# pitlover/Monocular-Depth-Estimation

Measured on AMD Instinct MI355X. Metric: images/sec (train step) NYU 640x480 bs=8/GPU, higher is better.
Workload: dtype fp32; 1 GPU; NewCRFs Swin-L (large07) train step, NYU 480x640; model=NewCRFs-L07, global_batch=8, per_gpu_batch=8, num_accum=1, parallelism=dp1, reference_config=json/nyu/newcrfs/newcrfs_github_eval.json, matmul_precision=fp32, hipgraph=False

## Files before the change

### monocular-depth-estimation_amd/csrc/winattn.hip

```cpp
#include "common.h"

namespace mdemi {

struct WinGeom {
  int B, H, W, Hp, Wp, nWh, nWw, shift, heads;
};

template <int WS>
struct Win {
  int b, wy, wx;
  __device__ Win(const WinGeom& g, int win) {
    wx = win % g.nWw;
    const int t = win / g.nWw;
    wy = t % g.nWh;
    b = t / g.nWh;
  }
  __device__ int row(const WinGeom& g, int t) const {
    const int py = wy * WS + t / WS, px = wx * WS + t % WS;
    int oy = py + g.shift, ox = px + g.shift;
    if (oy >= g.Hp) oy -= g.Hp;
    if (ox >= g.Wp) ox -= g.Wp;
    if (oy >= g.H || ox >= g.W) return -1;
    return (b * g.H + oy) * g.W + ox;
  }
  __device__ int region(const WinGeom& g, int t) const {
    const int py = wy * WS + t / WS, px = wx * WS + t % WS;
    const int rh = py < g.Hp - WS ? 0 : (py < g.Hp - g.shift ? 1 : 2);
    const int rw = px < g.Wp - WS ? 0 : (px < g.Wp - g.shift ? 1 : 2);
    return rh * 3 + rw;
  }
};

template <int WS>
__device__ __forceinline__ int rpb_index(int i, int j) {
  return (i / WS - j / WS + WS - 1) * (2 * WS - 1) + (i % WS - j % WS + WS - 1);
}

template <int HD>
__device__ __forceinline__ void load_row(float4 (&dst)[HD / 4], const float* src) {
#pragma unroll
  for (int q = 0; q < HD / 4; ++q) dst[q] = reinterpret_cast<const float4*>(src)[q];
}

__device__ __forceinline__ float4 ld_tok4(const float* base, int64_t ld, int row, const float* pad, int off) {
  if (row >= 0) return *reinterpret_cast<const float4*>(base + (int64_t)row * ld + off);
  if (pad) return *reinterpret_cast<const float4*>(pad + off);
  return make_float4(0.f, 0.f, 0.f, 0.f);
}

__device__ float g_wa_zero[128];

__device__ __forceinline__ const float* tok_src(const float* base, int64_t ld, int row, const float* pad, bool real) {
  const float* padsrc = pad ? pad : g_wa_zero;
  return !real ? g_wa_zero : (row >= 0 ? base + (int64_t)row * ld : padsrc);
}

__device__ __forceinline__ float dot4(const float4& a, const float4& b) {
  return fmaf(a.x, b.x, fmaf(a.y, b.y, fmaf(a.z, b.z, a.w * b.w)));
}

struct WinParams {
  WinGeom g;
  float scale;
  const float* q; const float* k; int64_t qk_ld;
  const float* q_pad; const float* k_pad;
  const float* v; int64_t v_ld; const float* v_pad;
  const float* rpb;
  float* out; int64_t out_ld;
  float* lse;
  const float* dout;
  float* dq; float* dk; int64_t dqk_ld;
  float* dv; int64_t dv_ld;
  float* partial;
  int off32;
  const float* live;
};

constexpr int WA_WAVES = 4, WA_NP = 64, WA_HD = 32, WA_N = 49, WA_T = 169;
typedef float wa_f16x __attribute__((ext_vector_type(16)));

__device__ __forceinline__ float f4c(const float4& v, int c) {
  return c == 0 ? v.x : (c == 1 ? v.y : (c == 2 ? v.z : v.w));
}
__device__ __forceinline__ wa_f16x mfma32(float a, float b, wa_f16x c) {
  return __builtin_amdgcn_mfma_f32_32x32x2f32(a, b, c, 0, 0, 0);
}
__device__ __forceinline__ int acc_row(int r, int h) { return (r & 3) + 8 * (r >> 2) + 4 * h; }

__device__ __forceinline__ void load_frag(float4 (&f)[4], const float* base, int64_t ld, int row, const float* pad,
                                          bool real, int col0, int h, float scale) {
  const float* src = tok_src(base, ld, row, pad, real);
  src = src == g_wa_zero ? src : src + col0;
#pragma unroll
  for (int g4 = 0; g4 < 4; ++g4) {
    float4 v = *reinterpret_cast<const float4*>(src + 8 * g4 + 4 * h);
    v.x *= scale; v.y *= scale; v.z *= scale; v.w *= scale;
    f[g4] = v;
  }
}

__device__ __forceinline__ void load_bias(wa_f16x (&acc)[2][2], const float* img, int lane) {
#pragma unroll
  for (int a = 0; a < 2; ++a)
#pragma unroll
    for (int b = 0; b < 2; ++b) {
      const float4* src = reinterpret_cast<const float4*>(img + ((a * 2 + b) * 64 + lane) * 16);
#pragma unroll
      for (int q4 = 0; q4 < 4; ++q4) {
        const float4 v = src[q4];
        acc[a][b][4 * q4 + 0] = v.x; acc[a][b][4 * q4 + 1] = v.y;
        acc[a][b][4 * q4 + 2] = v.z; acc[a][b][4 * q4 + 3] = v.w;
      }
    }
}

__device__ __forceinline__ void mma_hd(wa_f16x (&acc)[2][2], const float4 (&fa)[2][4], const float4 (&fb)[2][4]) {
#pragma unroll
  for (int g4 = 0; g4 < 4; ++g4)
#pragma unroll
    for (int c = 0; c < 4; ++c)
#pragma unroll
      for (int a = 0; a < 2; ++a)
#pragma unroll
        for (int b = 0; b < 2; ++b) acc[a][b] = mfma32(f4c(fa[a][g4], c), f4c(fb[b][g4], c), acc[a][b]);
}

__device__ __forceinline__ void mma_tok(wa_f16x (&out)[2], const float (*rows)[WA_HD], const wa_f16x (&acc)[2][2],
                                        int l31, int h) {
#pragma unroll
  for (int t = 0; t < 2; ++t)
#pragma unroll
    for (int s = 0; s < (t == 0 ? 16 : 12); ++s) {
      const float a = rows[t * 32 + acc_row(s, h)][l31];
#pragma unroll
      for (int n = 0; n < 2; ++n) out[n] = mfma32(a, acc[t][n][s], out[n]);
    }
}

__device__ __forceinline__ void wave_lds_sync() {
  __builtin_amdgcn_fence(__ATOMIC_RELEASE, "wavefront");
  __builtin_amdgcn_wave_barrier();
  __builtin_amdgcn_fence(__ATOMIC_ACQUIRE, "wavefront");
}

struct WaItem {
  int item, win, hh;
};
__device__ __forceinline__ WaItem wa_item(const WinParams& p) {
  WaItem it;
  it.item = blockIdx.x * WA_WAVES + (threadIdx.x >> 6);
  it.win = it.item / p.g.heads;
  it.hh = it.item % p.g.heads;
  return it;
}

__device__ __forceinline__ bool wa_dead(const WinParams& p, int b) { return p.live && p.live[b] == 0.f; }
__device__ __forceinline__ void wa_zero_rows(const WinGeom& g, const Win<7>& w, float* base, int64_t ld, int col0,
                                             int lane) {
  for (int e = lane; e < WA_N * (WA_HD / 4); e += 64) {
    const int row = w.row(g, e >> 3);
    if (row >= 0)
      *reinterpret_cast<float4*>(base + (int64_t)row * ld + col0 + 4 * (e & 7)) = make_float4(0.f, 0.f, 0.f, 0.f);
  }
}

__device__ __forceinline__ bool wa_regions(const WinParams& p, const Win<7>& w, int8_t* reg, int lane) {
  const bool border = p.g.shift > 0 && (w.wy == p.g.nWh - 1 || w.wx == p.g.nWw - 1);
  if (border) reg[lane] = lane < WA_N ? (int8_t)w.region(p.g, lane) : (int8_t)0;
  return border;
}

template <int WS, int HD>
__global__ __launch_bounds__(256) void winattn_fwd_kernel(WinParams p, const float* __restrict__ biasT, int nitems) {
  static_assert(WS == 7 && HD == WA_HD, "MFMA window attention is built for 7x7 windows, head_dim 32");
  __shared__ float Vs[WA_WAVES][WA_NP][WA_HD];
  __shared__ int8_t regs[WA_WAVES][WA_NP];
  const WinGeom& g = p.g;
  const int lane = threadIdx.x & 63, wv = threadIdx.x >> 6, l31 = lane & 31, h = lane >> 5;
  const WaItem it = wa_item(p);
  if (it.item >= nitems) return;
  const Win<WS> w(g, it.win);
  const int col0 = it.hh * HD;
  if (wa_dead(p, w.b)) {
    wa_zero_rows(g, w, p.out, p.out_ld, col0, lane);
    if (p.lse && lane < WA_N) p.lse[(int64_t)it.item * WA_N + lane] = 0.f;
    return;
  }
  for (int e = lane; e < WA_NP * HD / 4; e += 64) {
    const int tok = e >> 3, c4 = e & 7;
    const float4 v = tok < WA_N ? ld_tok4(p.v, p.v_ld, w.row(g, tok), p.v_pad, col0 + 4 * c4)
                                : make_float4(0.f, 0.f, 0.f, 0.f);
    *reinterpret_cast<float4*>(&Vs[wv][tok][4 * c4]) = v;
  }
  const bool border = wa_regions(p, w, regs[wv], lane);
  wa_f16x s[2][2];
  load_bias(s, biasT + (size_t)it.hh * 4096, lane);
  {
    float4 kf[2][4], qf[2][4];
#pragma unroll
    for (int t = 0; t < 2; ++t) {
      const int tok = t * 32 + l31;
      const bool real = tok < WA_N;
      const int row = real ? w.row(g, tok) : -1;
      load_frag(kf[t], p.k, p.qk_ld, row, p.k_pad, real, col0, h, 1.f);
      load_frag(qf[t], p.q, p.qk_ld, row, p.q_pad, real, col0, h, p.scale);
    }
    mma_hd(s, kf, qf);
  }
  wave_lds_sync();
  if (border) {
#pragma unroll
    for (int n = 0; n < 2; ++n) {
      const int rq = regs[wv][n * 32 + l31];
#pragma unroll
      for (int t = 0; t < 2; ++t)
#pragma unroll
        for (int r = 0; r < 16; ++r)
          if (regs[wv][t * 32 + acc_row(r, h)] != rq) s[t][n][r] -= 100.f;
    }
  }
  float lse[2];
#pragma unroll
  for (int n = 0; n < 2; ++n) {
    float m = -INFINITY;
#pragma unroll
    for (int t = 0; t < 2; ++t)
#pragma unroll
      for (int r = 0; r < 16; ++r) m = fmaxf(m, s[t][n][r]);
    m = fmaxf(m, __shfl_xor(m, 32, 64));
    float l = 0.f;
#pragma unroll
    for (int t = 0; t < 2; ++t)
#pragma unroll
      for (int r = 0; r < 16; ++r) {
        const float e = __expf(s[t][n][r] - m);
        s[t][n][r] = e;
        l += e;
      }
    l += __shfl_xor(l, 32, 64);
    const float inv = 1.f / l;
#pragma unroll
    for (int t = 0; t < 2; ++t)
#pragma unroll
      for (int r = 0; r < 16; ++r) s[t][n][r] *= inv;
    lse[n] = m + __logf(l);
  }
  wa_f16x o[2];
#pragma unroll
  for (int n = 0; n < 2; ++n)
#pragma unroll
    for (int r = 0; r < 16; ++r) o[n][r] = 0.f;
  mma_tok(o, Vs[wv], s, l31, h);
#pragma unroll
  for (int n = 0; n < 2; ++n) {
    const int q = n * 32 + l31;
    if (q >= WA_N) continue;
    const int row = w.row(g, q);
    if (p.lse && h == 0) p.lse[(int64_t)it.item * WA_N + q] = row >= 0 ? lse[n] : INFINITY;
    if (row < 0) continue;
    float* dst = p.out + (int64_t)row * p.out_ld + col0;
#pragma unroll
    for (int a = 0; a < 4; ++a)
      *reinterpret_cast<float4*>(dst + 8 * a + 4 * h) =
          make_float4(o[n][4 * a], o[n][4 * a + 1], o[n][4 * a + 2], o[n][4 * a + 3]);
  }
}

#ifdef WA_OCC3
constexpr int WA_TR = 56, WA_TP = 57;
#else
constexpr int WA_TR = WA_NP, WA_TP = WA_NP + 1;
#endif

__device__ __forceinline__ float col_val(const float* base, int64_t ld, const float* pad, int row, int col) {
  const float* src = row >= 0 ? base + (int64_t)row * ld + col : ((row == -1 && pad) ? pad + col : g_wa_zero + (col & 31));
  return *src;
}

__host__ __device__ constexpr int key_tab(int key) { return (key / 7) * 13 + key % 7; }

__host__ __device__ constexpr int acc_tok_kind(int ti, int r) {
  return (ti * 32 + (r & 3) + 8 * (r >> 2) + 4 >= WA_N) ? ((ti * 32 + (r & 3) + 8 * (r >> 2) >= WA_N) ? 2 : 1) : 0;
}
__host__ __device__ constexpr int pair_tok_kind(int j) { return 2 * j + 1 >= WA_N ? (2 * j >= WA_N ? 2 : 1) : 0; }

template <bool FAST>
__device__ __forceinline__ void fetch_pairs(float (&c)[25], const float* base, int64_t ld, const float* pad,
                                            const int* rt, int col0, int l31, int h, float scale) {
  if (FAST) {
    const float* cb = base + col0 + l31;
#pragma unroll
    for (int j = 0; j < 25; ++j) {
      const int kind = pair_tok_kind(j);
      const float v = cb[__umul24((unsigned)rt[kind ? 2 * j : 2 * j + h], (unsigned)ld)];
      c[j] = (kind && h) ? 0.f : scale * v;
    }
  } else {
#pragma unroll
    for (int j = 0; j < 25; ++j) c[j] = scale * col_val(base, ld, pad, rt[2 * j + h], col0 + l31);
  }
}

template <bool FAST>
__device__ __forceinline__ void fetch_keys(float (&c)[2][16], const float* base, int64_t ld, const float* pad,
                                           const int* rt, int col0, int l31, int h) {
  if (FAST) {
    const float* cb = base + col0 + l31;
#pragma unroll
    for (int t = 0; t < 2; ++t)
#pragma unroll
      for (int r = 0; r < 16; ++r) {
        const int kind = acc_tok_kind(t, r);
        if (kind == 2) {
          c[t][r] = 0.f;
          continue;
        }
        const float v = cb[__umul24((unsigned)rt[kind ? t * 32 + acc_row(r, 0) : t * 32 + acc_row(r, h)], (unsigned)ld)];
        c[t][r] = (kind && h) ? 0.f : v;
      }
  } else {
#pragma unroll
    for (int t = 0; t < 2; ++t)
#pragma unroll
      for (int r = 0; r < 16; ++r) c[t][r] = col_val(base, ld, pad, rt[t * 32 + acc_row(r, h)], col0 + l31);
  }
}

template <int WS, int HD>
#ifdef WA_OCC3
#define WA_BWD_OCC 3
#else
#define WA_BWD_OCC 2
#endif
__global__ __launch_bounds__(256) __attribute__((amdgpu_waves_per_eu(WA_BWD_OCC, WA_BWD_OCC))) void winattn_bwd_kernel(
    WinParams p, const float* __restrict__ biasT, int nitems) {
  __shared__ float tbuf[WA_WAVES][WA_TR][WA_TP];
  __shared__ float padk[WA_WAVES][WA_HD], padv[WA_WAVES][WA_HD];
  __shared__ int8_t regs[WA_WAVES][WA_NP];
  __shared__ int rowtab[WA_WAVES][WA_NP];
  const WinGeom& g = p.g;
  const int lane = threadIdx.x & 63, wv = threadIdx.x >> 6, l31 = lane & 31, h = lane >> 5;
  const WaItem it = wa_item(p);
  if (it.item >= nitems) return;
  const Win<WS> w(g, it.win);
  const int col0 = it.hh * HD;
  if (wa_dead(p, w.b)) {
    wa_zero_rows(g, w, p.dq, p.dqk_ld, col0, lane);
    wa_zero_rows(g, w, p.dk, p.dqk_ld, col0, lane);
    wa_zero_rows(g, w, p.dv, p.dv_ld, col0, lane);
    float* P = p.partial + (int64_t)it.item * (WA_T + 2 * HD);
    for (int e = lane; e < WA_T + 2 * HD; e += 64) P[e] = 0.f;
    return;
  }
  float lse[2];
#pragma unroll
  for (int n = 0; n < 2; ++n) {
    const int q = n * 32 + l31;
    lse[n] = (q < WA_N) ? p.lse[(int64_t)it.item * WA_N + q] : INFINITY;
  }
  const int myrow = lane < WA_N ? w.row(g, lane) : -2;
  rowtab[wv][lane] = myrow;
  if (lane < HD) { padk[wv][lane] = 0.f; padv[wv][lane] = 0.f; }
  const bool border = wa_regions(p, w, regs[wv], lane);
  const bool fast = p.off32 && __ballot(myrow == -1) == 0;

  wa_f16x s[2][2], dp[2][2];
  load_bias(s, biasT + (size_t)it.hh * 4096, lane);
  int trow[2];
  bool treal[2];
  {
    float4 kf[2][4], qf[2][4];
#pragma unroll
    for (int t = 0; t < 2; ++t) {
      const int tok = t * 32 + l31;
      treal[t] = tok < WA_N;
      trow[t] = treal[t] ? w.row(g, tok) : -1;
      load_frag(kf[t], p.k, p.qk_ld, trow[t], p.k_pad, treal[t], col0, h, 1.f);
      load_frag(qf[t], p.q, p.qk_ld, trow[t], p.q_pad, treal[t], col0, h, p.scale);
    }
    mma_hd(s, kf, qf);
  }
  wave_lds_sync();
  if (border) {
#pragma unroll
    for (int n = 0; n < 2; ++n) {
      const int rq = regs[wv][n * 32 + l31];
#pragma unroll
      for (int t = 0; t < 2; ++t)
#pragma unroll
        for (int r = 0; r < 16; ++r)
          if (regs[wv][t * 32 + acc_row(r, h)] != rq) s[t][n][r] -= 100.f;
    }
  }
#pragma unroll
  for (int n = 0; n < 2; ++n)
#pragma unroll
    for (int t = 0; t < 2; ++t)
#pragma unroll
      for (int r = 0; r < 16; ++r) s[t][n][r] = __expf(s[t][n][r] - lse[n]);
  auto to_lds = [&](const wa_f16x (&x)[2][2]) {
#pragma unroll
    for (int t = 0; t < 2; ++t)
#pragma unroll
      for (int n = 0; n < 2; ++n)
#pragma unroll
        for (int r = 0; r < 16; ++r) {
#ifdef WA_OCC3
          if (t * 32 + acc_row(r, 0) >= WA_TR || (n == 1 && l31 >= WA_TP - 32)) continue;
#endif
          tbuf[wv][t * 32 + acc_row(r, h)][n * 32 + l31] = x[t][n][r];
        }
  };
  auto key_side = [&](const float (&colv)[25], float* gbase, int64_t gld, float* padacc) {
    wa_f16x acc[2];
#pragma unroll
    for (int ti = 0; ti < 2; ++ti)
#pragma unroll
      for (int r = 0; r < 16; ++r) acc[ti][r] = 0.f;
#pragma unroll
    for (int j = 0; j < 25; ++j)
#pragma unroll
      for (int ti = 0; ti < 2; ++ti) acc[ti] = mfma32(tbuf[wv][ti * 32 + l31][2 * j + h], colv[j], acc[ti]);
    if (fast) {
      float* gb = gbase + col0 + l31;
      const int* rt = rowtab[wv];
#pragma unroll
      for (int ti = 0; ti < 2; ++ti)
#pragma unroll
        for (int r = 0; r < 16; ++r) {
          const int kind = acc_tok_kind(ti, r);
          if (kind == 2 || (kind == 1 && h)) continue;
          gb[__umul24((unsigned)rt[ti * 32 + acc_row(r, h)], (unsigned)gld)] = acc[ti][r];
        }
      return;
    }
#pragma unroll
    for (int ti = 0; ti < 2; ++ti)
#pragma unroll
      for (int r = 0; r < 16; ++r) {
        const int row = rowtab[wv][ti * 32 + acc_row(r, h)];
        if (row >= 0) gbase[(int64_t)row * gld + col0 + l31] = acc[ti][r];
        else if (row == -1) atomicAdd(&padacc[l31], acc[ti][r]);
      }
  };
  {
    to_lds(s);
    wave_lds_sync();
    float dc[25];
    if (fast) fetch_pairs<true>(dc, p.dout, p.out_ld, nullptr, rowtab[wv], col0, l31, h, 1.f);
    else fetch_pairs<false>(dc, p.dout, p.out_ld, nullptr, rowtab[wv], col0, l31, h, 1.f);
    key_side(dc, p.dv, p.dv_ld, padv[wv]);
  }
  float D[2];
  {
    float4 vf[2][4], df[2][4];
#pragma unroll
    for (int t = 0; t < 2; ++t) {
      const bool qo = treal[t] && trow[t] >= 0;
      load_frag(vf[t], p.v, p.v_ld, trow[t], p.v_pad, treal[t], col0, h, 1.f);
      load_frag(df[t], p.dout, p.out_ld, trow[t], nullptr, qo, col0, h, 1.f);
      float4 of[4];
      load_frag(of, p.out, p.out_ld, trow[t], nullptr, qo, col0, h, 1.f);
      float part = 0.f;
#pragma unroll
      for (int g4 = 0; g4 < 4; ++g4) part += dot4(df[t][g4], of[g4]);
      D[t] = part + __shfl_xor(part, 32, 64);
    }
#pragma unroll
    for (int a = 0; a < 2; ++a)
#pragma unroll
      for (int b = 0; b < 2; ++b)
#pragma unroll
        for (int r = 0; r < 16; ++r) dp[a][b][r] = 0.f;
    mma_hd(dp, vf, df);
  }
#pragma unroll
  for (int n = 0; n < 2; ++n)
#pragma unroll
    for (int t = 0; t < 2; ++t)
#pragma unroll
      for (int r = 0; r < 16; ++r) {
        float pr;
#ifdef WA_OCC3
        if (t * 32 + acc_row(r, 0) >= WA_TR) pr = 0.f;
        else if (n == 1) pr = l31 < WA_TP - 32 ? tbuf[wv][t * 32 + acc_row(r, h)][32 + min(l31, WA_TP - 33)] : 0.f;
        else
#endif
        pr = tbuf[wv][t * 32 + acc_row(r, h)][n * 32 + l31];
        dp[t][n][r] = pr * (dp[t][n][r] - D[n]);
      }
  float kc[2][16];
  if (fast) fetch_keys<true>(kc, p.k, p.qk_ld, p.k_pad, rowtab[wv], col0, l31, h);
  else fetch_keys<false>(kc, p.k, p.qk_ld, p.k_pad, rowtab[wv], col0, l31, h);
  wave_lds_sync();
  to_lds(dp);
  wave_lds_sync();
  float qc[25];
  if (fast) fetch_pairs<true>(qc, p.q, p.qk_ld, p.q_pad, rowtab[wv], col0, l31, h, p.scale);
  else fetch_pairs<false>(qc, p.q, p.qk_ld, p.q_pad, rowtab[wv], col0, l31, h, p.scale);
  {
    wa_f16x dq[2];
#pragma unroll
    for (int n = 0; n < 2; ++n)
#pragma unroll
      for (int r = 0; r < 16; ++r) dq[n][r] = 0.f;
#pragma unroll
    for (int t = 0; t < 2; ++t)
#pragma unroll
      for (int r = 0; r < (t == 0 ? 16 : 12); ++r)
#pragma unroll
        for (int n = 0; n < 2; ++n)
          dq[n] = mfma32(kc[t][r], tbuf[wv][t * 32 + acc_row(r, h)][n * 32 + l31], dq[n]);
#pragma unroll
    for (int n = 0; n < 2; ++n) {
      if (!treal[n] || trow[n] < 0) continue;
      float* dst = p.dq + (int64_t)trow[n] * p.dqk_ld + col0;
#pragma unroll
      for (int a = 0; a < 4; ++a)
        *reinterpret_cast<float4*>(dst + 8 * a + 4 * h) =
            make_float4(dq[n][4 * a] * p.scale, dq[n][4 * a + 1] * p.scale, dq[n][4 * a + 2] * p.scale,
                        dq[n][4 * a + 3] * p.scale);
    }
  }
  key_side(qc, p.dk, p.dqk_ld, padk[wv]);
  float E[13];
#pragma unroll
  for (int e = 0; e < 13; ++e) E[e] = 0.f;
  const int sky = lane / WS, sqy = lane - sky * WS;
  if (lane < WA_N) {
    const float* blk = &tbuf[wv][sky * WS][sqy * WS];
#pragma unroll
    for (int kx = 0; kx < WS; ++kx)
#pragma unroll
      for (int qx = 0; qx < WS; ++qx) E[qx - kx + WS - 1] += blk[kx * WA_TP + qx];
  }
  wave_lds_sync();
  constexpr int ND = 2 * WS - 1;
  float* Eb = &tbuf[wv][0][0];
  if (lane < WA_N) {
#pragma unroll
    for (int e = 0; e < ND; ++e) Eb[lane * ND + e] = E[e];
  }
  wave_lds_sync();
  float* P = p.partial + (int64_t)it.item * (WA_T + 2 * HD);
  for (int e = lane; e < WA_T; e += 64) {
    const int dy = e / ND - (WS - 1), dxi = e % ND;
    const int ky0 = max(0, -dy), ky1 = min(WS - 1, WS - 1 - dy);
    float acc = 0.f;
    for (int ky = ky0; ky <= ky1; ++ky) acc += Eb[(ky * WS + ky + dy) * ND + dxi];
    P[e] = acc;
  }
  if (lane < HD) {
    P[WA_T + lane] = padk[wv][lane];
    P[WA_T + HD + lane] = padv[wv][lane];
  }
}

__global__ __launch_bounds__(256) void wa_bias_kernel(const float* __restrict__ rpb, int heads, float* biasT,
                                                      float* biasN) {
  const int e = blockIdx.x * 256 + threadIdx.x;
  if (e >= heads * 4096) return;
  const int hh = e >> 12, rem = e & 4095;
  const int tile = rem >> 10, lane = (rem >> 4) & 63, r = rem & 15;
  const int row = (tile >> 1) * 32 + acc_row(r, lane >> 5), col = (tile & 1) * 32 + (lane & 31);
  auto val = [&](int q, int key) {
    if (key >= WA_N) return -INFINITY;
    if (q >= WA_N) return 0.f;
    return rpb[rpb_index<7>(q, key) * heads + hh];
  };
  if (biasT) biasT[e] = val(col, row);
  if (biasN) biasN[e] = val(row, col);
}

template <int WS, int HD>
__global__ void winattn_bwd_scatter(const float* __restrict__ sums, int heads, float* d_rpb, float* dk_pad,
                                    float* dv_pad, float* dq_pad) {
  constexpr int T = (2 * WS - 1) * (2 * WS - 1), R = T + 2 * HD;
  const int e = blockIdx.x * blockDim.x + threadIdx.x;
  if (e >= heads * R) return;
  const int h = e / R, t = e % R;
  const float s = sums[e];
  if (t < T) d_rpb[t * heads + h] = s;
  else if (t < T + HD) { if (dk_pad) dk_pad[h * HD + t - T] = s; }
  else if (dv_pad) dv_pad[h * HD + t - T - HD] = s;
  if (dq_pad && t < HD) dq_pad[h * HD + t] = 0.f;
}

static int make_params(const mdemi_winattn_desc* d, WinParams& p, int& nwin) {
  MDEMI_REQUIRE(d, "winattn: null descriptor");
  MDEMI_REQUIRE(d->B > 0 && d->H > 0 && d->W > 0 && d->heads > 0, "winattn: bad sizes");
  MDEMI_REQUIRE(d->window == 7 && d->head_dim == 32, "winattn: only window 7 / head_dim 32 are built (got %d/%d)",
                d->window, d->head_dim);
  MDEMI_REQUIRE(d->shift >= 0 && d->shift < d->window, "winattn: bad shift %d", d->shift);
  MDEMI_REQUIRE(d->q && d->k && d->v && d->rpb_table, "winattn: null input");
  MDEMI_REQUIRE(d->qk_ld % 4 == 0 && d->v_ld % 4 == 0 && d->out_ld % 4 == 0, "winattn: row strides must be %% 4");
  const int ws = d->window;
  p.g.B = d->B; p.g.H = d->H; p.g.W = d->W;
  p.g.Hp = (d->H + ws - 1) / ws * ws; p.g.Wp = (d->W + ws - 1) / ws * ws;
  p.g.nWh = p.g.Hp / ws; p.g.nWw = p.g.Wp / ws;
  p.g.shift = d->shift; p.g.heads = d->heads;
  p.scale = d->scale;
  p.q = d->q; p.k = d->k; p.qk_ld = d->qk_ld; p.q_pad = d->q_pad; p.k_pad = d->k_pad;
  p.v = d->v; p.v_ld = d->v_ld; p.v_pad = d->v_pad;
  p.rpb = d->rpb_table;
  p.out = d->out; p.out_ld = d->out_ld;
  p.lse = d->lse;
  p.dout = d->dout; p.dq = d->dq; p.dk = d->dk; p.dqk_ld = d->dqk_ld; p.dv = d->dv; p.dv_ld = d->dv_ld;
  p.partial = (float*)d->workspace;
  p.live = d->sample_live;
  {
    const int64_t rows = (int64_t)d->B * d->H * d->W;
    const int64_t lds[4] = {d->qk_ld, d->out_ld, d->dqk_ld, d->dv_ld};
    bool ok = rows < (1 << 24);
    for (int64_t ld : lds) ok = ok && ld >= 0 && ld < (1 << 24) && rows * ld < (int64_t(1) << 32);
    p.off32 = ok;
  }
  nwin = d->B * p.g.nWh * p.g.nWw;
  return MDEMI_OK;
}

}

using namespace mdemi;

static int wa_items(const mdemi_winattn_desc* d, int nwin) { return nwin * d->heads; }
static size_t wa_bias_bytes(const mdemi_winattn_desc* d) { return (size_t)d->heads * 4096 * sizeof(float); }

extern "C" size_t mdemi_winattn_fwd_workspace_size(const mdemi_winattn_desc* d) {
  WinParams p;
  int nwin;
  if (make_params(d, p, nwin)) return 0;
  return wa_bias_bytes(d);
}

extern "C" int mdemi_winattn_fwd(const mdemi_winattn_desc* d, void* stream) {
  WinParams p;
  int nwin;
  int rc = make_params(d, p, nwin);
  if (rc) return rc;
  MDEMI_REQUIRE(d->out, "winattn_fwd: null out");
  if (!d->workspace || (size_t)d->workspace_bytes < wa_bias_bytes(d)) {
    set_error("winattn_fwd: needs %zu workspace bytes", wa_bias_bytes(d));
    return MDEMI_EWORKSPACE;
  }
  hipStream_t st = (hipStream_t)stream;
  float* biasT = (float*)d->workspace;
  hipLaunchKernelGGL(wa_bias_kernel, dim3(d->heads * 16), dim3(256), 0, st, d->rpb_table, d->heads, biasT,
                     (float*)nullptr);
  const int nitems = wa_items(d, nwin);
  hipLaunchKernelGGL((winattn_fwd_kernel<7, 32>), dim3(cdiv(nitems, WA_WAVES)), dim3(64 * WA_WAVES), 0, st, p,
                     (const float*)biasT, nitems);
  return check_launch("winattn_fwd");
}

static size_t wa_part_bytes(int items, int R) { return align_up((size_t)items * R * 4, 256); }
extern "C" size_t mdemi_winattn_bwd_workspace_size(const mdemi_winattn_desc* d) {
  WinParams p;
  int nwin;
  if (make_params(d, p, nwin)) return 0;
  const int R = WA_T + 2 * WA_HD;
  const int items = wa_items(d, nwin);
  return wa_part_bytes(items, R) + wa_bias_bytes(d) + align_up((size_t)d->heads * R * 4, 256) +
         colsum_ws_bytes(nwin, (int64_t)d->heads * R);
}

extern "C" int mdemi_winattn_bwd(const mdemi_winattn_desc* d, void* stream) {
  return mdemi_winattn_bwd_bias(d, nullptr, stream);
}

extern "C" int mdemi_winattn_bwd_bias(const mdemi_winattn_desc* d, const float* bias_expanded, void* stream) {
  WinParams p;
  int nwin;
  int rc = make_params(d, p, nwin);
  if (rc) return rc;
  MDEMI_REQUIRE(d->dout && d->dq && d->dk && d->dv && d->d_rpb_table, "winattn_bwd: null gradient buffer");
  MDEMI_REQUIRE(d->out && d->lse, "winattn_bwd: needs the forward output and its saved lse");
  MDEMI_REQUIRE(d->dqk_ld % 4 == 0 && d->dv_ld % 4 == 0, "winattn_bwd: gradient strides must be %% 4");
  const size_t need = mdemi_winattn_bwd_workspace_size(d);
  if (!d->workspace || (size_t)d->workspace_bytes < need) {
    set_error("winattn_bwd: needs %zu workspace bytes", need);
    return MDEMI_EWORKSPACE;
  }
  hipStream_t st = (hipStream_t)stream;
  const int R = WA_T + 2 * WA_HD;
  const int items = wa_items(d, nwin);
  char* ws = (char*)d->workspace;
  p.partial = (float*)ws;
  float* biasT = (float*)(ws + wa_part_bytes(items, R));
  float* sums = (float*)((char*)biasT + wa_bias_bytes(d));
  void* cws = (char*)sums + align_up((size_t)d->heads * R * 4, 256);
  if (bias_expanded)
    biasT = const_cast<float*>(bias_expanded);
  else
    hipLaunchKernelGGL(wa_bias_kernel, dim3(d->heads * 16), dim3(256), 0, st, d->rpb_table, d->heads, biasT,
                       (float*)nullptr);
  hipLaunchKernelGGL((winattn_bwd_kernel<7, 32>), dim3((unsigned)cdiv(items, WA_WAVES)), dim3(64 * WA_WAVES), 0, st,
                     p, (const float*)biasT, items);
  int rc2 = colsum_launch(p.partial, nwin, (int64_t)d->heads * R, (int64_t)d->heads * R, sums, 0, cws, st);
  if (rc2) return rc2;
  hipLaunchKernelGGL((winattn_bwd_scatter<7, 32>), dim3((d->heads * R + 255) / 256), dim3(256), 0, st, sums, d->heads,
                     d->d_rpb_table, d->dk_pad, d->dv_pad, d->dq_pad);
  return check_launch("winattn_bwd");
}
```

Measured before the change: 63.34 images/sec.

## Transpose window-attention LDS score/V tiles for vectorized conflict-free MFMA operand reads

Stores the forward V tile transposed with a padded pitch so the P·V MFMA loop reads four k-steps per 16-byte LDS load, with explicit sched_group_barrier interleaving. In backward, the score image uses a permuted column layout so key-side reductions also use float4 loads. Global loads of dout, out, k and q are hoisted earlier to overlap with compute, dq reuses register-resident dp instead of re-reading LDS, and a barrier is dropped. A fused column-sum plus scatter finish kernel replaces the two-kernel reduction when the window count is small. Forward occupancy is pinned to 3 waves per EU, which caps register use and may add spills.

```diff
diff --git a/monocular-depth-estimation_amd/csrc/winattn.hip b/monocular-depth-estimation_amd/csrc/winattn.hip
--- a/monocular-depth-estimation_amd/csrc/winattn.hip
+++ b/monocular-depth-estimation_amd/csrc/winattn.hip
@@ -1,4 +1,5 @@
 #include "common.h"
+#include "winattn_layout.h"
 
 namespace mdemi {
 
@@ -40,12 +41,6 @@
 __device__ __forceinline__ void load_row(float4 (&dst)[HD / 4], const float* src) {
 #pragma unroll
   for (int q = 0; q < HD / 4; ++q) dst[q] = reinterpret_cast<const float4*>(src)[q];
-}
-
-__device__ __forceinline__ float4 ld_tok4(const float* base, int64_t ld, int row, const float* pad, int off) {
-  if (row >= 0) return *reinterpret_cast<const float4*>(base + (int64_t)row * ld + off);
-  if (pad) return *reinterpret_cast<const float4*>(pad + off);
-  return make_float4(0.f, 0.f, 0.f, 0.f);
 }
 
 __device__ float g_wa_zero[128];
@@ -85,7 +80,7 @@
 __device__ __forceinline__ wa_f16x mfma32(float a, float b, wa_f16x c) {
   return __builtin_amdgcn_mfma_f32_32x32x2f32(a, b, c, 0, 0, 0);
 }
-__device__ __forceinline__ int acc_row(int r, int h) { return (r & 3) + 8 * (r >> 2) + 4 * h; }
+__host__ __device__ constexpr int acc_row(int r, int h) { return (r & 3) + 8 * (r >> 2) + 4 * h; }
 
 __device__ __forceinline__ void load_frag(float4 (&f)[4], const float* base, int64_t ld, int row, const float* pad,
                                           bool real, int col0, int h, float scale) {
@@ -125,22 +120,32 @@
         for (int b = 0; b < 2; ++b) acc[a][b] = mfma32(f4c(fa[a][g4], c), f4c(fb[b][g4], c), acc[a][b]);
 }
 
-__device__ __forceinline__ void mma_tok(wa_f16x (&out)[2], const float (*rows)[WA_HD], const wa_f16x (&acc)[2][2],
-                                        int l31, int h) {
-#pragma unroll
-  for (int t = 0; t < 2; ++t)
-#pragma unroll
-    for (int s = 0; s < (t == 0 ? 16 : 12); ++s) {
-      const float a = rows[t * 32 + acc_row(s, h)][l31];
-#pragma unroll
-      for (int n = 0; n < 2; ++n) out[n] = mfma32(a, acc[t][n][s], out[n]);
-    }
+__device__ __forceinline__ void mma_tok(wa_f16x (&out)[2], const float (*rowsT)[WA_IMG_PITCH],
+                                        const wa_f16x (&acc)[2][2], int l31, int h) {
+  static_assert(acc_row(4, 0) == 8 && acc_row(3, 1) == 7, "steps 4g..4g+3 of half h: tokens 8g + 4h + 0..3");
+  const float4* arow = reinterpret_cast<const float4*>(&rowsT[l31][4 * h]);
+  constexpr int NG = 7;
+  float4 cur = arow[0], nxt;
+  __builtin_amdgcn_sched_group_barrier(0x100, 1, 0);
+#pragma unroll
+  for (int g4 = 0; g4 < NG; ++g4) {
+    if (g4 + 1 < NG) nxt = arow[2 * (g4 + 1)];
+#pragma unroll
+    for (int c = 0; c < 4; ++c)
+#pragma unroll
+      for (int n = 0; n < 2; ++n) out[n] = mfma32(f4c(cur, c), acc[g4 >> 2][n][4 * (g4 & 3) + c], out[n]);
+    if (g4 + 1 < NG) {
+      __builtin_amdgcn_sched_group_barrier(0x100, 1, 0);
+      __builtin_amdgcn_sched_group_barrier(0x008, 8, 0);
+    }
+    cur = nxt;
+  }
 }
 
 __device__ __forceinline__ void wave_lds_sync() {
-  __builtin_amdgcn_fence(__ATOMIC_RELEASE, "wavefront");
+  __builtin_amdgcn_fence(__ATOMIC_RELEASE, "wavefront", "local");
   __builtin_amdgcn_wave_barrier();
-  __builtin_amdgcn_fence(__ATOMIC_ACQUIRE, "wavefront");
+  __builtin_amdgcn_fence(__ATOMIC_ACQUIRE, "wavefront", "local");
 }
 
 struct WaItem {
@@ -171,9 +176,10 @@
 }
 
 template <int WS, int HD>
-__global__ __launch_bounds__(256) void winattn_fwd_kernel(WinParams p, const float* __restrict__ biasT, int nitems) {
+__global__ __launch_bounds__(256) __attribute__((amdgpu_waves_per_eu(3, 3))) void winattn_fwd_kernel(
+    WinParams p, const float* __restrict__ biasT, int nitems) {
   static_assert(WS == 7 && HD == WA_HD, "MFMA window attention is built for 7x7 windows, head_dim 32");
-  __shared__ float Vs[WA_WAVES][WA_NP][WA_HD];
+  __shared__ __attribute__((aligned(16))) float Vs[WA_WAVES][WA_HD][WA_IMG_PITCH];
   __shared__ int8_t regs[WA_WAVES][WA_NP];
   const WinGeom& g = p.g;
   const int lane = threadIdx.x & 63, wv = threadIdx.x >> 6, l31 = lane & 31, h = lane >> 5;
@@ -186,16 +192,15 @@
     if (p.lse && lane < WA_N) p.lse[(int64_t)it.item * WA_N + lane] = 0.f;
     return;
   }
-  for (int e = lane; e < WA_NP * HD / 4; e += 64) {
-    const int tok = e >> 3, c4 = e & 7;
-    const float4 v = tok < WA_N ? ld_tok4(p.v, p.v_ld, w.row(g, tok), p.v_pad, col0 + 4 * c4)
-                                : make_float4(0.f, 0.f, 0.f, 0.f);
-    *reinterpret_cast<float4*>(&Vs[wv][tok][4 * c4]) = v;
-  }
   const bool border = wa_regions(p, w, regs[wv], lane);
   wa_f16x s[2][2];
-  load_bias(s, biasT + (size_t)it.hh * 4096, lane);
   {
+    float4 vrow[HD / 4];
+    {
+      const bool real = lane < WA_N;
+      const float* src = tok_src(p.v, p.v_ld, real ? w.row(g, lane) : -1, p.v_pad, real);
+      load_row<HD>(vrow, src == g_wa_zero ? src : src + col0);
+    }
     float4 kf[2][4], qf[2][4];
 #pragma unroll
     for (int t = 0; t < 2; ++t) {
@@ -204,6 +209,12 @@
       const int row = real ? w.row(g, tok) : -1;
       load_frag(kf[t], p.k, p.qk_ld, row, p.k_pad, real, col0, h, 1.f);
       load_frag(qf[t], p.q, p.qk_ld, row, p.q_pad, real, col0, h, p.scale);
+    }
+    load_bias(s, biasT + (size_t)it.hh * 4096, lane);
+#pragma unroll
+    for (int q4 = 0; q4 < HD / 4; ++q4) {
+      Vs[wv][4 * q4 + 0][lane] = vrow[q4].x; Vs[wv][4 * q4 + 1][lane] = vrow[q4].y;
+      Vs[wv][4 * q4 + 2][lane] = vrow[q4].z; Vs[wv][4 * q4 + 3][lane] = vrow[q4].w;
     }
     mma_hd(s, kf, qf);
   }
@@ -266,11 +277,8 @@
   }
 }
 
-#ifdef WA_OCC3
-constexpr int WA_TR = 56, WA_TP = 57;
-#else
-constexpr int WA_TR = WA_NP, WA_TP = WA_NP + 1;
-#endif
+constexpr int WA_TR = WA_IMG_ROWS, WA_TP = WA_IMG_PITCH;
+static_assert(WA_TR == WA_NP && WA_KSTEPS == (WA_N + 1) / 2, "score image: 64 keys, 25 query pairs");
 
 __device__ __forceinline__ float col_val(const float* base, int64_t ld, const float* pad, int row, int col) {
   const float* src = row >= 0 ? base + (int64_t)row * ld + col : ((row == -1 && pad) ? pad + col : g_wa_zero + (col & 31));
@@ -327,14 +335,9 @@
 }
 
 template <int WS, int HD>
-#ifdef WA_OCC3
-#define WA_BWD_OCC 3
-#else
-#define WA_BWD_OCC 2
-#endif
-__global__ __launch_bounds__(256) __attribute__((amdgpu_waves_per_eu(WA_BWD_OCC, WA_BWD_OCC))) void winattn_bwd_kernel(
+__global__ __launch_bounds__(256) __attribute__((amdgpu_waves_per_eu(2, 2))) void winattn_bwd_kernel(
     WinParams p, const float* __restrict__ biasT, int nitems) {
-  __shared__ float tbuf[WA_WAVES][WA_TR][WA_TP];
+  __shared__ __attribute__((aligned(16))) float tbuf[WA_WAVES][WA_TR][WA_TP];
   __shared__ float padk[WA_WAVES][WA_HD], padv[WA_WAVES][WA_HD];
   __shared__ int8_t regs[WA_WAVES][WA_NP];
   __shared__ int rowtab[WA_WAVES][WA_NP];
@@ -363,11 +366,13 @@
   if (lane < HD) { padk[wv][lane] = 0.f; padv[wv][lane] = 0.f; }
   const bool border = wa_regions(p, w, regs[wv], lane);
   const bool fast = p.off32 && __ballot(myrow == -1) == 0;
+  wave_lds_sync();
 
   wa_f16x s[2][2], dp[2][2];
   load_bias(s, biasT + (size_t)it.hh * 4096, lane);
   int trow[2];
   bool treal[2];
+  float dc[25];
   {
     float4 kf[2][4], qf[2][4];
 #pragma unroll
@@ -378,9 +383,10 @@
       load_frag(kf[t], p.k, p.qk_ld, trow[t], p.k_pad, treal[t], col0, h, 1.f);
       load_frag(qf[t], p.q, p.qk_ld, trow[t], p.q_pad, treal[t], col0, h, p.scale);
     }
+    if (fast) fetch_pairs<true>(dc, p.dout, p.out_ld, nullptr, rowtab[wv], col0, l31, h, 1.f);
+    else fetch_pairs<false>(dc, p.dout, p.out_ld, nullptr, rowtab[wv], col0, l31, h, 1.f);
     mma_hd(s, kf, qf);
   }
-  wave_lds_sync();
   if (border) {
 #pragma unroll
     for (int n = 0; n < 2; ++n) {
@@ -398,18 +404,15 @@
     for (int t = 0; t < 2; ++t)
 #pragma unroll
       for (int r = 0; r < 16; ++r) s[t][n][r] = __expf(s[t][n][r] - lse[n]);
+  const int pc0 = wa_pcol(l31);
+  static_assert(wa_pcol(32) == 16 && wa_pcol(33) == wa_pcol(1) + 16, "query tile 1 sits 16 columns after tile 0");
   auto to_lds = [&](const wa_f16x (&x)[2][2]) {
 #pragma unroll
     for (int t = 0; t < 2; ++t)
 #pragma unroll
       for (int n = 0; n < 2; ++n)
 #pragma unroll
-        for (int r = 0; r < 16; ++r) {
-#ifdef WA_OCC3
-          if (t * 32 + acc_row(r, 0) >= WA_TR || (n == 1 && l31 >= WA_TP - 32)) continue;
-#endif
-          tbuf[wv][t * 32 + acc_row(r, h)][n * 32 + l31] = x[t][n][r];
-        }
+        for (int r = 0; r < 16; ++r) tbuf[wv][t * 32 + acc_row(r, h)][pc0 + 16 * n] = x[t][n][r];
   };
   auto key_side = [&](const float (&colv)[25], float* gbase, int64_t gld, float* padacc) {
     wa_f16x acc[2];
@@ -417,10 +420,31 @@
     for (int ti = 0; ti < 2; ++ti)
 #pragma unroll
       for (int r = 0; r < 16; ++r) acc[ti][r] = 0.f;
-#pragma unroll
-    for (int j = 0; j < 25; ++j)
-#pragma unroll
-      for (int ti = 0; ti < 2; ++ti) acc[ti] = mfma32(tbuf[wv][ti * 32 + l31][2 * j + h], colv[j], acc[ti]);
+    const float4* arow[2] = {reinterpret_cast<const float4*>(&tbuf[wv][l31][wa_group_col(0, h)]),
+                             reinterpret_cast<const float4*>(&tbuf[wv][32 + l31][wa_group_col(0, h)])};
+    constexpr int NG = (WA_KSTEPS + 3) / 4;
+    float4 cur[2] = {arow[0][0], arow[1][0]}, nxt[2];
+    __builtin_amdgcn_sched_group_barrier(0x100, 2, 0);
+#pragma unroll
+    for (int g4 = 0; g4 < NG; ++g4) {
+      if (g4 + 1 < NG) {
+        nxt[0] = arow[0][g4 + 1];
+        nxt[1] = arow[1][g4 + 1];
+      }
+#pragma unroll
+      for (int c = 0; c < 4; ++c) {
+        const int j = 4 * g4 + c;
+        if (j >= WA_KSTEPS) continue;
+#pragma unroll
+        for (int ti = 0; ti < 2; ++ti) acc[ti] = mfma32(f4c(cur[ti], c), colv[j], acc[ti]);
+      }
+      if (g4 + 1 < NG) {
+        __builtin_amdgcn_sched_group_barrier(0x100, 2, 0);
+        __builtin_amdgcn_sched_group_barrier(0x008, 8, 0);
+      }
+      cur[0] = nxt[0];
+      cur[1] = nxt[1];
+    }
     if (fast) {
       float* gb = gbase + col0 + l31;
       const int* rt = rowtab[wv];
@@ -443,27 +467,32 @@
         else if (row == -1) atomicAdd(&padacc[l31], acc[ti][r]);
       }
   };
+  to_lds(s);
+  wave_lds_sync();
+  float D[2];
+  float kc[2][16], qc[25];
   {
-    to_lds(s);
-    wave_lds_sync();
-    float dc[25];
-    if (fast) fetch_pairs<true>(dc, p.dout, p.out_ld, nullptr, rowtab[wv], col0, l31, h, 1.f);
-    else fetch_pairs<false>(dc, p.dout, p.out_ld, nullptr, rowtab[wv], col0, l31, h, 1.f);
-    key_side(dc, p.dv, p.dv_ld, padv[wv]);
-  }
-  float D[2];
-  {
-    float4 vf[2][4], df[2][4];
+    float4 vf[2][4], df[2][4], of[2][4];
 #pragma unroll
     for (int t = 0; t < 2; ++t) {
       const bool qo = treal[t] && trow[t] >= 0;
       load_frag(vf[t], p.v, p.v_ld, trow[t], p.v_pad, treal[t], col0, h, 1.f);
       load_frag(df[t], p.dout, p.out_ld, trow[t], nullptr, qo, col0, h, 1.f);
-      float4 of[4];
-      load_frag(of, p.out, p.out_ld, trow[t], nullptr, qo, col0, h, 1.f);
+      load_frag(of[t], p.out, p.out_ld, trow[t], nullptr, qo, col0, h, 1.f);
+    }
+    key_side(dc, p.dv, p.dv_ld, padv[wv]);
+    if (fast) {
+      fetch_keys<true>(kc, p.k, p.qk_ld, p.k_pad, rowtab[wv], col0, l31, h);
+      fetch_pairs<true>(qc, p.q, p.qk_ld, p.q_pad, rowtab[wv], col0, l31, h, p.scale);
+    } else {
+      fetch_keys<false>(kc, p.k, p.qk_ld, p.k_pad, rowtab[wv], col0, l31, h);
+      fetch_pairs<false>(qc, p.q, p.qk_ld, p.q_pad, rowtab[wv], col0, l31, h, p.scale);
+    }
+#pragma unroll
+    for (int t = 0; t < 2; ++t) {
       float part = 0.f;
 #pragma unroll
-      for (int g4 = 0; g4 < 4; ++g4) part += dot4(df[t][g4], of[g4]);
+      for (int g4 = 0; g4 < 4; ++g4) part += dot4(df[t][g4], of[t][g4]);
       D[t] = part + __shfl_xor(part, 32, 64);
     }
 #pragma unroll
@@ -477,27 +506,15 @@
 #pragma unroll
   for (int n = 0; n < 2; ++n)
 #pragma unroll
-    for (int t = 0; t < 2; ++t)
-#pragma unroll
-      for (int r = 0; r < 16; ++r) {
-        float pr;
-#ifdef WA_OCC3
-        if (t * 32 + acc_row(r, 0) >= WA_TR) pr = 0.f;
-        else if (n == 1) pr = l31 < WA_TP - 32 ? tbuf[wv][t * 32 + acc_row(r, h)][32 + min(l31, WA_TP - 33)] : 0.f;
-        else
-#endif
-        pr = tbuf[wv][t * 32 + acc_row(r, h)][n * 32 + l31];
-        dp[t][n][r] = pr * (dp[t][n][r] - D[n]);
-      }
-  float kc[2][16];
-  if (fast) fetch_keys<true>(kc, p.k, p.qk_ld, p.k_pad, rowtab[wv], col0, l31, h);
-  else fetch_keys<false>(kc, p.k, p.qk_ld, p.k_pad, rowtab[wv], col0, l31, h);
+    for (int t = 0; t < 2; ++t) {
+      float pr[16];
+#pragma unroll
+      for (int r = 0; r < 16; ++r) pr[r] = tbuf[wv][t * 32 + acc_row(r, h)][pc0 + 16 * n];
+#pragma unroll
+      for (int r = 0; r < 16; ++r) dp[t][n][r] = pr[r] * (dp[t][n][r] - D[n]);
+    }
   wave_lds_sync();
   to_lds(dp);
-  wave_lds_sync();
-  float qc[25];
-  if (fast) fetch_pairs<true>(qc, p.q, p.qk_ld, p.q_pad, rowtab[wv], col0, l31, h, p.scale);
-  else fetch_pairs<false>(qc, p.q, p.qk_ld, p.q_pad, rowtab[wv], col0, l31, h, p.scale);
   {
     wa_f16x dq[2];
 #pragma unroll
@@ -510,7 +527,7 @@
       for (int r = 0; r < (t == 0 ? 16 : 12); ++r)
 #pragma unroll
         for (int n = 0; n < 2; ++n)
-          dq[n] = mfma32(kc[t][r], tbuf[wv][t * 32 + acc_row(r, h)][n * 32 + l31], dq[n]);
+          dq[n] = mfma32(kc[t][r], dp[t][n][r], dq[n]);
 #pragma unroll
     for (int n = 0; n < 2; ++n) {
       if (!treal[n] || trow[n] < 0) continue;
@@ -522,17 +539,20 @@
                         dq[n][4 * a + 3] * p.scale);
     }
   }
+  wave_lds_sync();
   key_side(qc, p.dk, p.dqk_ld, padk[wv]);
   float E[13];
 #pragma unroll
   for (int e = 0; e < 13; ++e) E[e] = 0.f;
   const int sky = lane / WS, sqy = lane - sky * WS;
   if (lane < WA_N) {
-    const float* blk = &tbuf[wv][sky * WS][sqy * WS];
+    const int q0 = sqy * WS, e0 = q0 & 1;
+    const float* row0 = &tbuf[wv][sky * WS][0];
+    const float* blk[2] = {row0 + e0 * 32 + (q0 >> 1), row0 + (1 - e0) * 32 + (q0 >> 1) + e0};
 #pragma unroll
     for (int kx = 0; kx < WS; ++kx)
 #pragma unroll
-      for (int qx = 0; qx < WS; ++qx) E[qx - kx + WS - 1] += blk[kx * WA_TP + qx];
+      for (int qx = 0; qx < WS; ++qx) E[qx - kx + WS - 1] += blk[qx & 1][kx * WA_TP + (qx >> 1)];
   }
   wave_lds_sync();
   constexpr int ND = 2 * WS - 1;
@@ -583,6 +603,39 @@
   if (t < T) d_rpb[t * heads + h] = s;
   else if (t < T + HD) { if (dk_pad) dk_pad[h * HD + t - T] = s; }
   else if (dv_pad) dv_pad[h * HD + t - T - HD] = s;
+  if (dq_pad && t < HD) dq_pad[h * HD + t] = 0.f;
+}
+
+constexpr int WA_FINISH_ROWS = 1024;
+template <int WS, int HD>
+__global__ __launch_bounds__(1024) void winattn_bwd_finish(const float* __restrict__ partial, int rows, int heads,
+                                                           float* d_rpb, float* dk_pad, float* dv_pad, float* dq_pad) {
+  constexpr int T = (2 * WS - 1) * (2 * WS - 1), R = T + 2 * HD;
+  __shared__ float red[32][33];
+  const int tx = threadIdx.x & 31, ty = threadIdx.x >> 5;
+  const int cols = heads * R, c = blockIdx.x * 32 + tx;
+  float s = 0.f;
+  if (c < cols) {
+    constexpr int NL = WA_FINISH_ROWS / 32;
+    float v[NL];
+#pragma unroll
+    for (int j = 0; j < NL; ++j) {
+      const int r = ty + 32 * j;
+      v[j] = r < rows ? partial[(int64_t)r * cols + c] : 0.f;
+    }
+#pragma unroll
+    for (int j = 0; j < NL; ++j) s += v[j];
+  }
+  red[ty][tx] = s;
+  __syncthreads();
+  if (ty != 0 || c >= cols) return;
+  float sum = 0.f;
+#pragma unroll
+  for (int k = 0; k < 32; ++k) sum += red[k][tx];
+  const int h = c / R, t = c % R;
+  if (t < T) d_rpb[t * heads + h] = sum;
+  else if (t < T + HD) { if (dk_pad) dk_pad[h * HD + t - T] = sum; }
+  else if (dv_pad) dv_pad[h * HD + t - T - HD] = sum;
   if (dq_pad && t < HD) dq_pad[h * HD + t] = 0.f;
 }
 
@@ -696,6 +749,11 @@
                        (float*)nullptr);
   hipLaunchKernelGGL((winattn_bwd_kernel<7, 32>), dim3((unsigned)cdiv(items, WA_WAVES)), dim3(64 * WA_WAVES), 0, st,
                      p, (const float*)biasT, items);
+  if (nwin <= WA_FINISH_ROWS && colsum_ws_bytes(nwin, (int64_t)d->heads * R) == 0) {
+    hipLaunchKernelGGL((winattn_bwd_finish<7, 32>), dim3((d->heads * R + 31) / 32), dim3(1024), 0, st,
+                       (const float*)p.partial, nwin, d->heads, d->d_rpb_table, d->dk_pad, d->dv_pad, d->dq_pad);
+    return check_launch("winattn_bwd");
+  }
   int rc2 = colsum_launch(p.partial, nwin, (int64_t)d->heads * R, (int64_t)d->heads * R, sums, 0, cws, st);
   if (rc2) return rc2;
   hipLaunchKernelGGL((winattn_bwd_scatter<7, 32>), dim3((d->heads * R + 255) / 256), dim3(256), 0, st, sums, d->heads,
diff --git a/monocular-depth-estimation_amd/csrc/winattn_layout.h b/monocular-depth-estimation_amd/csrc/winattn_layout.h
--- /dev/null
+++ b/monocular-depth-estimation_amd/csrc/winattn_layout.h
@@ -0,0 +1,46 @@
+#pragma once
+
+namespace mdemi {
+
+constexpr int WA_IMG_ROWS = 64;
+constexpr int WA_IMG_PITCH = 68;
+constexpr int WA_KSTEPS = 25;
+
+constexpr int wa_pcol(int q) { return (q & 1) * 32 + (q >> 1); }
+constexpr int wa_group_col(int g, int h) { return h * 32 + 4 * g; }
+
+namespace wa_layout_check {
+constexpr bool bijection() {
+  bool seen[64] = {};
+  for (int q = 0; q < 64; ++q) {
+    const int p = wa_pcol(q);
+    if (p < 0 || p >= 64 || seen[p]) return false;
+    seen[p] = true;
+  }
+  return true;
+}
+constexpr bool groups_are_ksteps() {
+  for (int h = 0; h < 2; ++h)
+    for (int j = 0; j < 32; ++j)
+      if (wa_pcol(2 * j + h) != wa_group_col(j >> 2, h) + (j & 3)) return false;
+  return true;
+}
+constexpr bool reads_conflict_free() {
+  bool seen[64] = {};
+  for (int row = 0; row < 16; ++row)
+    for (int c = 0; c < 4; ++c) {
+      const int b = (row * WA_IMG_PITCH + c) % 64;
+      if (seen[b]) return false;
+      seen[b] = true;
+    }
+  return true;
+}
+}
+
+static_assert(WA_IMG_PITCH % 4 == 0 && WA_IMG_PITCH >= 64, "16-byte aligned rows that hold 64 queries");
+static_assert(wa_layout_check::bijection(), "wa_pcol is a permutation of 0..63");
+static_assert(wa_layout_check::groups_are_ksteps(), "one 16-byte read = k-steps 4g..4g+3 = queries (2j, 2j+1) by half");
+static_assert(wa_layout_check::reads_conflict_free(), "16 rows of a lane group cover the 64 banks once");
+static_assert(WA_KSTEPS <= 4 * 7 &&2 * (WA_KSTEPS - 1) + 1 < 64, "seven reads per row cover the 25 k-steps");
+
+}
```

After: 63.55 images/sec (median of 6 runs). About the same (+0.3%).
